# usamireko/WFL-ASR

Measured on AMD Instinct MI355X. Metric: audio_seconds_labeled_per_sec_per_node, higher is better.
Workload: dtype bf16; 1 GPU; BASELINE configs[1]: openai/whisper-base + 2 Conformer blocks, 16 x 30 s clips per GPU; clips_per_gpu=16, frames_per_clip=1500, tags=141, parallelism=clip-sharded dp1, launch=eager, batches_in_flight=2

## Files before the change

### include/wfl_asr.h

```cpp
#ifndef WFL_ASR_H
#define WFL_ASR_H

#include <stdint.h>

#ifdef __cplusplus
extern "C" {
#endif

typedef struct wfl_model wfl_model;

#define WFL_ENC_WHISPER 0
#define WFL_ENC_WAVLM 1
#define WFL_ENC_NONE 2

#define WFL_ABI_VERSION 2

typedef struct wfl_arch {
  int32_t abi_version;
  int32_t encoder_type;
  int32_t d_model;
  int32_t enc_layers;
  int32_t enc_heads;
  int32_t enc_ffn;
  int32_t n_mels;
// ... 63 lines not shown
int32_t wfl_head(wfl_model* m, const float* hidden, int32_t B, int32_t T, const int32_t* lang_id, int32_t lang_mode,
                 float threshold, void* workspace, int64_t workspace_bytes, int32_t* ids, int32_t* argmax, float* maxprob,
                 float* offsets, float* logits, int32_t* status, void* stream);

int32_t wfl_check(wfl_model* m, void* workspace, int64_t workspace_bytes, int32_t B, int32_t L, void* stream);


int32_t wfl_logmel(wfl_model* m, const float* wav, int64_t ldw, const int32_t* lens, int32_t B, int32_t L,
                   float* out, void* workspace, int64_t workspace_bytes, void* stream);

int32_t wfl_op_gemm(const void* A, int64_t lda, int32_t cin, int64_t tap_stride, const void* W, int32_t M, int32_t N,
                    int32_t K, int32_t n_valid, int32_t P, int32_t T, void* C, int64_t ldc, int64_t c_lead,
                    int32_t c_pitch, const float* bias, const void* res, int64_t ldres, float alpha, int32_t act,
                    int32_t glu, int32_t out_f32, void* stream);

int32_t wfl_op_gemm_split(const void* A_hi, const void* A_lo, int64_t lda, int32_t cin, int64_t tap_stride, const void* W3, int32_t M,
                          int32_t N, int32_t K, int32_t n_valid, int32_t P, int32_t T, void* C, void* C_lo, int64_t ldc,
                          int64_t c_lead, int32_t c_pitch, const float* bias, const void* res, const void* res_lo, int64_t ldres,
                          float alpha, int32_t act, int32_t glu, void* stream);

int32_t wfl_op_gemm_ln(const void* A, int64_t lda, const void* W, int32_t M, int32_t N, int32_t K, int32_t n_valid, int32_t P,
                       int32_t T, void* C, int64_t ldc, int64_t c_lead, int32_t c_pitch, const float* bias, const float* ln_s,
                       float ln_eps, int32_t act, void* stream);

int32_t wfl_op_attention(const void* QK, int64_t ldqk, int64_t lead, const void* V, int64_t ldv, void* O, int64_t ldo, int32_t B,
                         int32_t T, int32_t P, int32_t heads, int32_t d, void* stream);

int32_t wfl_op_attention_ex(const void* QK, const void* QK_lo, int64_t ldqk, int64_t lead, const void* V, const void* V_lo, int64_t ldv,
                            void* O, void* O_lo, int64_t ldo, int32_t B, int32_t T, int32_t P, int32_t heads, int32_t d, const float* bias,
                            const float* gate, const int32_t* clip_T, void* O8, void* O8_lo, int64_t ldo8, float o8_scale, int32_t* status,
// ... 218 lines not shown
```

### wfl-asr_amd/_lib.py

```python
from __future__ import annotations

import ctypes as C
import os

import numpy as np

PKG = os.path.dirname(os.path.abspath(__file__))
LIB_PATH = os.environ.get("WFL_LIB_PATH") or os.path.join(PKG, "libwfl_asr_hip.so")
ABI_VERSION = 2


class WflArch(C.Structure):
    _fields_ = [
        ("abi_version", C.c_int32), ("encoder_type", C.c_int32), ("d_model", C.c_int32), ("enc_layers", C.c_int32),
        ("enc_heads", C.c_int32), ("enc_ffn", C.c_int32), ("n_mels", C.c_int32), ("max_positions", C.c_int32),
        ("num_classes", C.c_int32), ("o_id", C.c_int32), ("num_languages", C.c_int32), ("lang_emb_dim", C.c_int32),
        ("enable_bilstm", C.c_int32), ("bilstm_layers", C.c_int32), ("n_conformer", C.c_int32),
        ("conformer_heads", C.c_int32), ("conformer_ff_expansion", C.c_int32), ("conformer_kernel", C.c_int32),
        ("enable_dilated", C.c_int32), ("dilated_depth", C.c_int32), ("dilated_kernel", C.c_int32),
        ("wavlm_n_conv", C.c_int32), ("wavlm_conv_dim", C.c_int32 * 8), ("wavlm_conv_kernel", C.c_int32 * 8),
        ("wavlm_conv_stride", C.c_int32 * 8), ("wavlm_group_norm", C.c_int32), ("wavlm_conv_bias", C.c_int32),
        ("wavlm_stable_layer_norm", C.c_int32), ("wavlm_pos_conv_kernel", C.c_int32),
        ("wavlm_pos_conv_groups", C.c_int32), ("wavlm_num_buckets", C.c_int32), ("wavlm_max_distance", C.c_int32),
        ("wavlm_do_normalize", C.c_int32), ("fp8_weights", C.c_int32), ("mel_hop", C.c_int32), ("precision", C.c_int32), ("fp8_activations", C.c_int32),
# ... 12 lines not shown
    "wfl_create": (_I, [C.POINTER(WflArch), C.POINTER(_P)]),
    "wfl_destroy": (None, [_P]),
    "wfl_load_tensor": (_I, [_P, C.c_char_p, _P, C.POINTER(_L), _I]),
    "wfl_finalize": (_I, [_P]),
    "wfl_num_frames": (_I, [_P, _I]),
    "wfl_workspace_bytes": (_L, [_P, _I, _I]),
    "wfl_device": (_I, [_P]),
    "wfl_set_average_languages": (_I, [_P, _P, _I]),
    "wfl_forward": (_I, [_P, _P, _L, _P, _I, _I, _P, _I, _F, _P, _L, _P, _P, _P, _P, _P, _P, _P, _P]),
    "wfl_encode": (_I, [_P, _P, _L, _P, _I, _I, _P, _L, _P, _P]),
    "wfl_head_workspace_bytes": (_L, [_P, _I, _I]),
    "wfl_head": (_I, [_P, _P, _I, _I, _P, _I, _F, _P, _L, _P, _P, _P, _P, _P, _P, _P]),
    "wfl_check": (_I, [_P, _P, _L, _I, _I, _P]),
    "wfl_logmel": (_I, [_P, _P, _L, _P, _I, _I, _P, _P, _L, _P]),
    "wfl_op_gemm": (_I, [_P, _L, _I, _L, _P, _I, _I, _I, _I, _I, _I, _P, _L, _L, _I, _P, _P, _L, _F, _I, _I, _I, _P]),
    "wfl_op_gemm_split": (_I, [_P, _P, _L, _I, _L, _P, _I, _I, _I, _I, _I, _I, _P, _P, _L, _L, _I, _P, _P, _P, _L, _F, _I, _I, _P]),
    "wfl_op_gemm_ln": (_I, [_P, _L, _P, _I, _I, _I, _I, _I, _I, _P, _L, _L, _I, _P, _P, _F, _I, _P]),
    "wfl_op_gemm_mx": (_I, [_P, _P, _L, _P, _P, _P, _F, _I, _I, _I, _I, _I, _P, _L, _L, _I, _P, _P, _P, _P, _F, _I, _P, _P, _L, _F, _P, _P]),
    "wfl_op_rows_fp8": (_I, [_P, _L, _P, _P, _P, _F, _L, _I, _I, _I, _I, _P, _P, _L, _P, _P]),
    "wfl_op_attention": (_I, [_P, _L, _L, _P, _L, _P, _L, _I, _I, _I, _I, _I, _P]),
    "wfl_op_attention_ex": (_I, [_P, _P, _L, _L, _P, _P, _L, _P, _P, _L, _I, _I, _I, _I, _I, _P, _P, _P, _P, _P, _L, _F, _P, _P]),
    "wfl_op_relpos_table": (_I, [_P, _P, _I, _I, _I, _P, _P]),
    "wfl_op_relpos_gate": (_I, [_P, _P, _L, _L, _I, _I, _I, _I, _I, _P, _P, _P, _P, _P]),
    "wfl_op_regroup": (_I, [_P, _I, _I, _I, _L, _L, _I, _I, _I, _P, _P, _P]),
    "wfl_op_wav_stats": (_I, [_P, _L, _P, _I, _I, _P, _P]),
    "wfl_op_clip_frames": (_I, [_P, _I, _I, _I, _P, _P, _I, _P, _P]),
    "wfl_op_conv0_scratch_bytes": (_L, [_I, _I, _I]),
    "wfl_op_conv0": (_I, [_P, _L, _P, _I, _I, _P, _P, _P, _P, _P, _I, _I, _P, _P, _L, _I, _I, _P, _L, _P]),
    "wfl_op_posconv": (_I, [_P, _L, _L, _I, _I, _I, _I, _I, _I, _P, _L, _P, _P, _P, _P, _P, _L, _P, _P]),
    "wfl_op_layernorm_act": (_I, [_P, _P, _L, _P, _P, _L, _P, _P, _F, _L, _I, _I, _I, _I, _I, _I, _P, _P]),
# ... 105 lines not shown
```

### wfl-asr_amd/csrc/common.h

```cpp
#pragma once
#include <hip/hip_runtime.h>
#include <stdint.h>

typedef __bf16 bf16_t;
typedef __attribute__((ext_vector_type(8))) __bf16 bf16x8;
typedef __attribute__((ext_vector_type(4))) __bf16 bf16x4;
typedef __attribute__((ext_vector_type(4))) float f32x4;
typedef __attribute__((ext_vector_type(16))) float f32x16;

#define WFL_ACT_NONE 0
#define WFL_ACT_GELU 1
#define WFL_ACT_RELU 2
#define WFL_ACT_SIGMOID 3

struct GemmArgs {
  const bf16_t* A;
  long lda;
  int cin;
  long tap_stride;
  int tap_wrap;
  long seg_off;
  const bf16_t* W;
  int M, N, K;
  int n_valid;
// ... 216 lines not shown
  bool need() {
    int d = 0;
    (void)hipGetDevice(&d);
    if ((mask >> (d & 31)) & 1u) return false;
    mask |= 1u << (d & 31);
    return true;
  }
};

int wfl_fail(int code, const char* msg);
int wfl_launch_gemm(const GemmArgs& a, hipStream_t s);
extern int g_wfl_gemm_kernel_id;
bool wfl_gemm_mx_takes(const GemmArgs& a);
int wfl_launch_gemm_mx(const GemmArgs& a, hipStream_t s);
bool wfl_gemm256_tri_takes(const GemmArgs& a);
bool wfl_gemm_stream_takes(const GemmArgs& a);
int wfl_launch_attention(const AttnArgs& a, hipStream_t s);
int wfl_launch_layernorm(const bf16_t* x, long ldx, bf16_t* y, long ldy, const float* g, const float* b, float eps,
                         long lead, int B, int P, int T, int C, hipStream_t s);
int wfl_launch_fill_i32(int* dst, long n, int value, hipStream_t s);
int wfl_launch_copy16(void* dst, const void* src, long bytes, hipStream_t s);
int wfl_launch_zero_halo(bf16_t* buf, long ld_bytes, long lead, int B, int P, int T, long tail_rows, hipStream_t s);
```

### wfl-asr_amd/csrc/gemm.hip

```cpp
#include "common.h"
#include <cstdlib>

#define BM 128
#define BN 128
#define BK 64
#define STAGE_BYTES (2 * BM * BK * 2)
#ifndef NSTAGE
#define NSTAGE 4
#endif
static_assert(NSTAGE >= 3 && NSTAGE <= 4, "the mid-iteration prefetch needs a ring of 3 or 4 K tiles");
#define EPI_BYTES (128 * 132 * 4)
#define LDS_BYTES (NSTAGE * STAGE_BYTES > EPI_BYTES ? NSTAGE * STAGE_BYTES : EPI_BYTES)

typedef __attribute__((address_space(1))) const void* gptr_t;
typedef __attribute__((address_space(3))) void* lptr_t;

#ifdef WFL_GEMM_STAMPS
#define STAMP(k) do { if (tid == 0 && p.stamps) p.stamps[(long)blockIdx.x * 8 + (k)] = __builtin_amdgcn_s_memrealtime(); } while (0)
#else
#define STAMP(k) do { } while (0)
#endif

static __device__ __forceinline__ void glds16(const bf16_t* g, char* l) {
  __builtin_amdgcn_global_load_lds((gptr_t)g, (lptr_t)l, 16, 0, 0);
// ... 290 lines not shown

int wfl_launch_gemm256(const GemmArgs& a, hipStream_t s);
int wfl_launch_gemm_stream(const GemmArgs& a, hipStream_t s);
bool wfl_gemm256_tri_takes(const GemmArgs& a);
bool wfl_gemm_stream_conv_takes(const GemmArgs& a);

static int tile_pref() {
  static int pref = -1;
  if (pref < 0) {
    const char* e = getenv("WFL_GEMM_TILE");
    pref = (e && atoi(e) == 128) ? 128 : 256;
  }
  return pref;
}

int wfl_launch_gemm(const GemmArgs& a, hipStream_t s) {
  if (a.M <= 0 || a.N <= 0 || a.N % BN || a.K <= 0 || a.K % BK || a.cin <= 0 || a.cin % BK || a.P <= 0 || a.P % 8 ||
      (!a.out_f32 && a.ldc % 8) || (a.res && a.ldres % 8) || (a.pos && a.ldpos % 8))
    return -1;
  if (a.a8 >= 2) {
    const int r = wfl_launch_gemm_mx(a, s);
    return r == 1 ? -1 : r;
  }
  if (tile_pref() == 256) {
    if (a.tap_wrap > 0 && wfl_gemm256_tri_takes(a) && !wfl_gemm_stream_conv_takes(a)) {
      static int tri_res = -1;
      if (tri_res < 0) { const char* e = getenv("WFL_TRI_RES"); tri_res = e ? atoi(e) : 1; }
      if (!a.res || tri_res) {
        const int r3 = wfl_launch_gemm256(a, s);
        if (r3 != 1) return r3;
      }
    }
    int r = wfl_launch_gemm_stream(a, s);
    if (r != 1) return r;
    if (a.ln_s || a.w8_scale) return -1;
    r = wfl_launch_gemm256(a, s);
    if (r != 1) return r;
  }
  if (a.ln_s || a.w8_scale) return -1;
  if (a.glu) {
    if (a.out_f32 || a.act != WFL_ACT_NONE) return -1;
    return launch_t<WFL_ACT_NONE, true, false>(a, s);
  }
  if (a.out_f32) {
    if (a.act == WFL_ACT_NONE) return launch_t<WFL_ACT_NONE, false, true>(a, s);
    if (a.act == WFL_ACT_SIGMOID) return launch_t<WFL_ACT_SIGMOID, false, true>(a, s);
// ... 11 lines not shown
```

### wfl-asr_amd/csrc/gemm_stream.hip

```cpp
#include "common.h"
#include <cstdlib>
#include <cstring>
#include <type_traits>

#define SBK 32
#ifndef SNST
#define SNST 4
#endif

#ifndef SNCU
#define SNCU 256
#endif

typedef __attribute__((address_space(1))) const void* sgptr_t;
typedef __attribute__((address_space(3))) void* slptr_t;
typedef __attribute__((ext_vector_type(2))) __bf16 bf16x2;

static __device__ __forceinline__ void sglds(const bf16_t* g, char* l) {
  __builtin_amdgcn_global_load_lds((sgptr_t)g, (slptr_t)l, 16, 0, 0);
}
static __device__ __forceinline__ int sswz(int row) { return (-(row >> 2)) & 3; }
static __device__ __forceinline__ int xswz(int row) { return ((row >> 2) & 1) << 1; }
#define XROT_ROWS 223
template <int N>
static __device__ __forceinline__ void wait_vm() { asm volatile("s_waitcnt vmcnt(%0)" ::"n"(N) : "memory"); }

#ifdef WFL_GEMM_STAMPS
#define SSTAMP(k) do { if (tid == 0 && p.stamps) { p.stamps[(long)blockIdx.x * 8 + (k)] = __builtin_amdgcn_s_memrealtime(); \
    if ((k) == 1) p.stamps[(long)blockIdx.x * 8 + 5] = __builtin_amdgcn_s_memtime(); \
    if ((k) == 2) p.stamps[(long)blockIdx.x * 8 + 6] = __builtin_amdgcn_s_memtime(); } } while (0)
#else
#define SSTAMP(k) do { } while (0)
#endif

template <int ACT, int MT, bool RES, int LNF, bool STATS, bool CONV, bool W8 = false, bool A8 = false, bool OUT8 = false, bool NOLO = false, bool ROT = false>
__global__ __launch_bounds__(512) void gemm_stream_kernel(GemmArgs p) {
  static_assert(!NOLO || CONV, "only the conv mode has an optional low half");
  static_assert(!ROT || CONV, "only the conv mode rotates frame fragments");
  static_assert(!CONV || (MT == 6 && !RES && LNF == 0 && !STATS), "conv mode: 192-row tiles, plain epilogue");
  static_assert(!W8 || (!CONV && MT == 6), "fp8 weights: plain 192-row mode");
  static_assert(!A8 || (!W8 && !CONV && MT == 6 && LNF == 0 && !STATS), "fp8 x fp8: the plain 192-row mode, no LayerNorm folding");
  static_assert(!OUT8 || (A8 && !RES), "fp8 output: the fp8 x fp8 kernel, no residual");
  constexpr int BMV = MT * 32;
#ifdef WFL_LAB_STB32
  constexpr int STB = 512 * SBK * 2;
  constexpr int WOFF = 256 * SBK * 2;
#else
  constexpr int STB = CONV ? 256 * SBK * 2 : BMV * SBK * 2 + 256 * SBK * (W8 ? 1 : 2);
  constexpr int WOFF = CONV ? 0 : BMV * SBK * 2;
#endif
  constexpr int AEXT = 224 * SBK * 2;
  constexpr int AOFF = SNST * STB;
  constexpr bool LOUT = RES || (CONV && !NOLO);
  constexpr int NSTORE = (LOUT ? 4 : 2) * MT + (STATS ? MT : 0);
  constexpr int SROW = 4;
  extern __shared__ __attribute__((aligned(16))) char smem[];
  float* stat_lds = (float*)(smem + SNST * STB + (CONV ? 2 * AEXT : 0));
  const int tid = threadIdx.x;
  const int lane = tid & 63;
  const int wid = __builtin_amdgcn_readfirstlane(tid >> 6);
  const int grp = wid >> 2, wq = wid & 3;
  const int g = lane >> 4, c = lane & 15;
  const int G = gridDim.x;

  SSTAMP(0);
  const int tiles_n = p.N / 256;
  const int tiles_m = (p.M + BMV - 1) / BMV;
  const int ntiles = tiles_m * tiles_n;
  const int nk = p.K / SBK;
// ... 132 lines not shown
      else if (SNST >= 5 && younger >= 3) { if (with_stores) wait_vm<3 * (L) + NSTORE>(); else wait_vm<3 * (L)>(); }  \
      else if (younger >= 2) { if (with_stores) wait_vm<2 * (L) + NSTORE>(); else wait_vm<2 * (L)>(); }              \
      else if (younger == 1) { if (with_stores) wait_vm<(L) + NSTORE>(); else wait_vm<(L)>(); }                      \
      else { if (with_stores) wait_vm<NSTORE>(); else wait_vm<0>(); }                                                \
    } while (0)
    if (CONV || two_x) WFL_WAITY(L2X); else WFL_WAITY(L1X);
#undef WFL_WAITY
  };

  int w_off[4];
#pragma unroll
  for (int v = 0; v < 4; ++v) {
#ifdef WFL_LAB_NOPERM
    const int r = wn + 16 * v + c;
#else
    const int r = wn + 32 * (v >> 1) + 8 * (c >> 2) + 4 * (v & 1) + (c & 3);
#endif
    w_off[v] = W8 ? WOFF + (r >> 3) * 256 + ((((r & 7) * 4 + g) ^ (((r >> 3) & 1) << 1) ^ (((r >> 4) & 1) << 4)) << 3)
                  : WOFF + r * 64 + ((g ^ sswz(r)) << 4);
  }
  const int x_off = wm * 64 + c * 64 + ((g ^ sswz(c)) << 4);

  f32x4 acc[MT][4];
#pragma unroll
  for (int u = 0; u < MT; ++u)
#pragma unroll
    for (int v = 0; v < 4; ++v) acc[u][v] = (f32x4){0.f, 0.f, 0.f, 0.f};
  float sa1 = 0.f, sa2 = 0.f, sb1 = 0.f, sb2 = 0.f;

  auto epilogue = [&](int m0, int n0) __attribute__((always_inline)) {
    const int nb = n0 + wn + 8 * g;
    constexpr int FCOL = ROT ? MT : 1, FROW = ROT ? 1 : 16;
    int mrow0 = m0 + wm + FCOL * c;
    int sidx_w = (((grp * 4 + wq) * (MT * 16)) + c) * 2, sidx_g = ((grp * 4 * (MT * 16)) + c) * 2, sidx_l = (grp * (MT * 16) + c) * 2;
    asm volatile("" : "+v"(mrow0), "+v"(sidx_w), "+v"(sidx_g), "+v"(sidx_l));
    f32x4 bj[4], sj[4], cj[(W8 || A8) ? 4 : 1];
#pragma unroll
    for (int h = 0; h < 2; ++h)
#pragma unroll
      for (int q = 0; q < 2; ++q) {
#ifdef WFL_ABL_EPI_NOLOAD
        bj[2 * h + q] = (f32x4){0.f, 0.f, 0.f, 0.f};
        if (LNF) sj[2 * h + q] = (f32x4){1.f, 1.f, 1.f, 1.f};
        if (W8 || A8) cj[2 * h + q] = (f32x4){1.f, 1.f, 1.f, 1.f};
#else
        bj[2 * h + q] = p.bias ? *(const f32x4*)(p.bias + nb + 32 * h + 4 * q) : (f32x4){0.f, 0.f, 0.f, 0.f};
        if (LNF) sj[2 * h + q] = *(const f32x4*)(p.ln_s + nb + 32 * h + 4 * q);
        if (W8 || A8) cj[2 * h + q] = *(const f32x4*)(p.w8_scale + nb + 32 * h + 4 * q);
#endif
      }
    float sa[A8 ? MT : 1];
    if (A8) {
#pragma unroll
      for (int u = 0; u < MT; ++u) {
        int m = mrow0 + FROW * u;
        m = m < p.M ? m : p.M - 1;
        sa[u] = p.a8_scale ? p.a8_scale[p.a8_lead + m] : p.a8_static;
      }
    }
    int P_ = p.P, cpitch = p.c_pitch;
    asm volatile("" : "+s"(P_), "+s"(cpitch));
    const float invP = __builtin_amdgcn_rcpf((float)P_);
    int orow[MT];
#pragma unroll
    for (int u = 0; u < MT; ++u) {
      const int m = mrow0 + FROW * u;
      int b = (int)((float)m * invP);
      int t = m - b * P_;
      if (t < 0) { t += P_; --b; }
      if (t >= P_) { t -= P_; ++b; }
      orow[u] = (m < p.M && t < p.T) ? (int)p.c_lead + b * cpitch + t : -1;
    }
    if (p.clip_T) {
#pragma unroll
      for (int u = 0; u < MT; ++u)
        if (orow[u] >= 0) {
          const int m = mrow0 + FROW * u;
          int b = (int)((float)m * invP);
          int t = m - b * P_;
          if (t < 0) { t += P_; --b; }
          if (t >= P_) { t -= P_; ++b; }
          if (t >= p.clip_T[b]) orow[u] = -1;
        }
    }
    constexpr int RING = 3;
    bf16x8 rr[RES ? RING : 1][2], rl[RES ? RING : 1][2];
    const bf16_t* res_lo = p.res_lo ? p.res_lo : p.res;
    const float lo_scale = p.res_lo ? 1.f : 0.f;
    auto load_res = [&](int u, int slot) __attribute__((always_inline)) {
      const long r = orow[u] >= 0 ? orow[u] : p.c_lead;
#pragma unroll
      for (int h = 0; h < 2; ++h) {
#ifdef WFL_ABL_EPI_NOLOAD
        rr[slot][h] = (bf16x8){0, 0, 0, 0, 0, 0, 0, 0}; rl[slot][h] = rr[slot][h]; (void)r;
#else
        rr[slot][h] = *(const bf16x8*)(p.res + r * p.ldres + nb + 32 * h);
        rl[slot][h] = *(const bf16x8*)(res_lo + r * p.ldres + nb + 32 * h);
#endif
      }
    };
    if (RES) {
#pragma unroll
      for (int u = 0; u < RING && u < MT; ++u) load_res(u, u);
    }
    float mu[LNF ? MT : 1], rs[LNF ? MT : 1];
    if (LNF == 1) {
#pragma unroll
      for (int u = 0; u < MT; ++u) {
        const float2 s = *(const float2*)(stat_lds + sidx_l + u * 32);
        mu[u] = s.x;
        rs[u] = s.y;
      }
    }
    if (LNF == 2) {
      f32x4 sp[MT][2];
#pragma unroll
      for (int u = 0; u < MT; ++u) {
        int m = mrow0 + FROW * u;
// ... 14 lines not shown
        mu[u] = mean;
        rs[u] = rsqrtf(fmaxf(__builtin_fmaf(-mean, mean, ex2), 0.f) + p.ln_eps);
      }
    }
    char* trash = (char*)p.trash + lane * 16;
#ifdef WFL_ABL_EPI_NOSTORE
#define WFL_KEEP(k) false
#else
#define WFL_KEEP(k) (k)
#endif
    float t1 = 0.f, t2 = 0.f;
    float amax8 = 0.f;
#pragma unroll
    for (int u = 0; u < MT; ++u) {
      __builtin_amdgcn_sched_barrier(0);
#pragma unroll
      for (int h = 0; h < 2; ++h) {
        float x[8];
#pragma unroll
        for (int q = 0; q < 2; ++q)
#pragma unroll
          for (int e = 0; e < 4; ++e) {
            float v = acc[u][2 * h + q][e];
            if (W8 || A8) v *= cj[2 * h + q][e];
            if (A8) v *= sa[u];
            if (LNF) v = (v - mu[u] * sj[2 * h + q][e]) * rs[u];
            if (ACT == WFL_ACT_GELU) {
              x[4 * q + e] = v + bj[2 * h + q][e];
              if (e & 1) {
                const f32x2 y = gelu_erf2((f32x2){x[4 * q + e - 1], x[4 * q + e]});
                x[4 * q + e - 1] = y[0]; x[4 * q + e] = y[1];
              }
              continue;
            }
            v = apply_act<ACT>(v + bj[2 * h + q][e]);
            if (RES) v = (bf2f(rr[u % RING][h][4 * q + e]) + lo_scale * bf2f(rl[u % RING][h][4 * q + e])) + p.alpha * v;
            x[4 * q + e] = v;
          }
        bf16x8 o;
#pragma unroll
        for (int e = 0; e < 8; ++e) o[e] = f2bf(x[e]);
        const bool keep = orow[u] >= 0 && nb + 32 * h < p.n_valid;
        if (OUT8) {
          int w0 = 0, w1 = 0;
          const float keepf = keep ? 1.f : 0.f;
#pragma unroll
          for (int e = 0; e < 8; ++e) {
            const float y = x[e] * p.c8_inv_scale;
            amax8 = fmaxf(amax8, fabsf(y) * keepf);
            x[e] = fminf(fmaxf(y, -448.f), 448.f);
          }
          w0 = __builtin_amdgcn_cvt_pk_fp8_f32(x[0], x[1], w0, false); w0 = __builtin_amdgcn_cvt_pk_fp8_f32(x[2], x[3], w0, true);
          w1 = __builtin_amdgcn_cvt_pk_fp8_f32(x[4], x[5], w1, false); w1 = __builtin_amdgcn_cvt_pk_fp8_f32(x[6], x[7], w1, true);
// ... 15 lines not shown
        }
        if (STATS) {
#pragma unroll
          for (int e = 0; e < 8; ++e) { const float r = bf2f(o[e]); t1 += r; t2 = fmaf(r, r, t2); }
        }
      }
      if (STATS) {
        t1 += __shfl_xor(t1, 16); t2 += __shfl_xor(t2, 16);
        t1 += __shfl_xor(t1, 32); t2 += __shfl_xor(t2, 32);
        if (g == 0) *(float2*)(stat_lds + sidx_w + u * 32) = float2{t1, t2};
        t1 = t2 = 0.f;
      }
#pragma unroll
      for (int v = 0; v < 4; ++v) acc[u][v] = (f32x4){0.f, 0.f, 0.f, 0.f};
      if (RES && u + RING < MT) load_res(u + RING, u % RING);
    }
    if (OUT8 && p.err) {
      if (__builtin_amdgcn_ballot_w64(amax8 > 448.f) && lane == 0) atomicOr(p.err, 2u);
    }
    if (STATS) {
      unsigned* cnt = (unsigned*)(stat_lds + 8 * (MT * 16) * 2) + grp;
      __builtin_amdgcn_s_waitcnt(0xC07F);
      unsigned ticket = 0;
      if (lane == 0) ticket = atomicAdd(cnt, 1u);
      ticket = __builtin_amdgcn_readfirstlane(ticket);
      const bool last = ticket == 3;
      if (last && lane == 0) *cnt = 0;
#pragma unroll
      for (int u = 0; u < MT; ++u) {
        float a1 = 0.f, a2 = 0.f;
// ... 185 lines not shown
#pragma unroll
    for (int kt = 1; kt < SNST - 2; ++kt) step_general(kt, std::false_type{});
    if (grp) steps_steady(std::true_type{}); else steps_steady(std::false_type{});
    for (int kt = nk - SNST > SNST - 2 ? nk - SNST : SNST - 2; kt < nk; ++kt) step_general(kt, std::false_type{});
    pm0 = m0; pn0 = n0;
    have_prev = true;
  }
  SSTAMP(2);
  SSTAMP(3);
  if (have_prev) epilogue(pm0, pn0);
  if (LNF == 1 && !grp) __builtin_amdgcn_s_barrier();
  SSTAMP(4);
#undef SSB
}

template <int ACT, int MT, bool RES, int LNF, bool STATS, bool CONV = false, bool W8 = false, bool A8 = false, bool OUT8 = false, bool NOLO = false, bool ROT = false>
static int launch_stream(const GemmArgs& a, hipStream_t s) {
  constexpr int BMV = MT * 32;
#ifdef WFL_LAB_STB32
  constexpr int lds = SNST * 512 * SBK * 2 + 8 * (MT * 16) * 2 * 4 + 64;
#else
  constexpr int lds = (CONV ? SNST * 256 * SBK * 2 + 2 * 224 * SBK * 2 : SNST * (BMV * SBK * 2 + 256 * SBK * (W8 ? 1 : 2))) + 8 * (MT * 16) * 2 * 4 + 64;
#endif
  const int tiles = ((a.M + BMV - 1) / BMV) * (a.N / 256);
  auto k = gemm_stream_kernel<ACT, MT, RES, LNF, STATS, CONV, W8, A8, OUT8, NOLO, ROT>;
  static WflOncePerDevice attr_once;
  if (attr_once.need()) {
    if (hipFuncSetAttribute((const void*)k, hipFuncAttributeMaxDynamicSharedMemorySize, lds) != hipSuccess) return -2;
  }
  g_wfl_gemm_kernel_id = CONV ? 6 : ((W8 || A8) ? 7 : (MT == 6 ? 1 : 5));
  hipLaunchKernelGGL(k, dim3(tiles < SNCU ? tiles : SNCU), dim3(512), lds, s, a);
  return hipGetLastError() == hipSuccess ? 0 : -3;
}

template <int ACT, bool RES, int LNF, bool STATS = false>
static int launch_stream_mt(const GemmArgs& a, hipStream_t s) {
  static int forced = -1;
  if (forced < 0) { const char* e = getenv("WFL_GEMM_BM"); forced = e ? atoi(e) : 0; }
#ifdef WFL_STREAM_MT8
  if (forced == 256) return launch_stream<ACT, 8, RES, LNF, STATS>(a, s);
// ... 18 lines not shown
  if (!g.c_lo) {
    switch (g.act) {
      case WFL_ACT_NONE: return launch_stream<WFL_ACT_NONE, 6, false, 0, false, true, false, false, false, true, ROT>(g, s);
      case WFL_ACT_GELU: return launch_stream<WFL_ACT_GELU, 6, false, 0, false, true, false, false, false, true, ROT>(g, s);
      case WFL_ACT_RELU: return launch_stream<WFL_ACT_RELU, 6, false, 0, false, true, false, false, false, true, ROT>(g, s);
    }
    return 1;
  }
  switch (g.act) {
    case WFL_ACT_NONE: return launch_stream<WFL_ACT_NONE, 6, false, 0, false, true, false, false, false, false, ROT>(g, s);
    case WFL_ACT_GELU: return launch_stream<WFL_ACT_GELU, 6, false, 0, false, true, false, false, false, false, ROT>(g, s);
    case WFL_ACT_RELU: return launch_stream<WFL_ACT_RELU, 6, false, 0, false, true, false, false, false, false, ROT>(g, s);
  }
  return 1;
}
bool wfl_gemm_stream_takes(const GemmArgs& a) {
  static int off = -1;
  if (off < 0) { const char* e = getenv("WFL_GEMM_NO_STREAM"); off = e && atoi(e) ? 1 : 0; }
  if (off) return false;
#ifdef WFL_LAB_NOSTREAM
  return false;
#endif
  if (a.glu || a.out_f32 || a.pos || a.clip_bias) return false;
  if (a.a8 >= 2) return false;
  if (a.tap_wrap > 0 && (a.ln_s || a.w8_scale || a.a8)) return false;
  if (a.c_lo && !a.res && !wfl_gemm_stream_conv(a)) return false;
  if (a.w8_scale && (a.cin < a.K || a.K % 64)) return false;
  if (a.a8 && (!a.w8_scale || a.ln_s || a.stats_out || a.stats_in || a.K % 128 || a.lda % 16 || a.K / 64 < 8 || (a.c8 && (a.res || a.ldc8 % 8))))
    return false;
  if (a.c8 && !a.a8) return false;
  if (a.N % 256 || a.K % SBK || a.cin % SBK || a.K / SBK < 8 || a.n_valid % 8) return false;
  if (a.stats_out && (!a.res || a.N / 256 > 4)) return false;
  if (a.stats_in && (!a.ln_s || a.stats_nsl <= 0 || a.stats_nsl > 4)) return false;
  if (a.res && a.act != WFL_ACT_NONE) return false;
  if (a.ln_s && (a.res || a.cin < a.K || (a.act != WFL_ACT_NONE && a.act != WFL_ACT_GELU))) return false;
  if (a.act == WFL_ACT_SIGMOID) return false;
  return true;
}


bool wfl_gemm_stream_conv_takes(const GemmArgs& a) { return wfl_gemm_stream_takes(a) && wfl_gemm_stream_conv(a); }

int wfl_launch_gemm_stream(const GemmArgs& a, hipStream_t s) {
  if (!wfl_gemm_stream_takes(a)) return 1;
  static void* trash[32] = {nullptr};
  int dev = 0;
  (void)hipGetDevice(&dev);
  dev &= 31;
  if (!trash[dev]) {
    if (hipMalloc(&trash[dev], 4096) != hipSuccess) return -2;
  }
  GemmArgs g = a;
  g.trash = trash[dev];
  g.ln_k_pow2 = (g.K & (g.K - 1)) == 0;
  g.ln_inv_k = g.ln_k_pow2 ? 1.0f / (float)g.K : 0.f;
  if (g.a8) {
    g.K /= 2; g.cin = g.K; g.lda /= 2;
    if (g.c8) return g.act == WFL_ACT_GELU ? launch_stream<WFL_ACT_GELU, 6, false, 0, false, false, false, true, true>(g, s) : -1;
    if (g.res) return g.act == WFL_ACT_NONE ? launch_stream<WFL_ACT_NONE, 6, true, 0, false, false, false, true>(g, s) : -1;
    if (g.act == WFL_ACT_NONE) return launch_stream<WFL_ACT_NONE, 6, false, 0, false, false, false, true>(g, s);
    return -1;
  }
  if (g.w8_scale) {
    if (g.ln_s && g.stats_in) {
      if (g.act == WFL_ACT_NONE) return launch_stream<WFL_ACT_NONE, 6, false, 2, false, false, true>(g, s);
      if (g.act == WFL_ACT_GELU) return launch_stream<WFL_ACT_GELU, 6, false, 2, false, false, true>(g, s);
      return -1;
    }
    if (g.res && !g.ln_s && g.act == WFL_ACT_NONE)
      return g.stats_out ? launch_stream<WFL_ACT_NONE, 6, true, 0, true, false, true>(g, s)
// ... 35 lines not shown
```

### wfl-asr_amd/csrc/model.hip

```cpp
#include "common.h"
#include "../../include/wfl_asr.h"

#include <cmath>
#include <cstdint>
#include <cstdio>
#include <cstring>
#include <map>
#include <set>
#include <string>
#include <vector>

int wfl_launch_logmel(const LogmelArgs& a, bf16_t* out, long ldo, long lead, int P, float* ref_out, hipStream_t s, bf16_t* out_lo = nullptr);
int wfl_launch_precise_finish(const PreciseFinishArgs& a, hipStream_t s);
int wfl_launch_melpower(const LogmelArgs& a, int hop, bf16_t* out, long ldo, long lead, int P, int split, int shift, hipStream_t s);

int wfl_launch_tag_decide(const TagArgs& a, hipStream_t s);
int wfl_launch_f32_to_rows(const float* in, bf16_t* x, long ldx, long lead, int B, int P, int T, int C, hipStream_t s, int split,
                           int shift, bf16_t* x_lo = nullptr);

int wfl_launch_lstm(LstmArgs a, void* exchange, hipStream_t s);

int wfl_launch_wav_stats(const float* wav, long ldw, int B, int L, double* stats, hipStream_t s, const int* lens = nullptr);
int wfl_launch_conv0(const Conv0Args& a, int group_norm, hipStream_t s);
int wfl_launch_clip_frames(const int* lens, int B, int L, int n, const int* kernel, const int* stride, int min_len, int* out, hipStream_t s);
// ... 1265 lines not shown
    void* const C = c.C;
    if (C == stats_for) stats_for = nullptr;
    const int B = r.M / r.P;
    const bf16_t* A_lo = lo_in(A);
    static int fused_on = -1;
    if (fused_on < 0) { const char* e = getenv("WFL_PRECISE_FUSED"); fused_on = e ? atoi(e) : 1; }
    static int pos_fused = -1;
    if (pos_fused < 0) { const char* e = getenv("WFL_PRECISE_POS_FUSED"); pos_fused = e ? atoi(e) : 1; }
    if (fused_on && W.W3 && A_lo && lo_of(C)) {
      GemmArgs g = gemm_args(A, lda, W, r, c, o);
      g.tap_wrap = W.K / g.cin; g.seg_off = (long)(A_lo - A);
      g.W = W.W3; g.K = 3 * W.K;
      g.res_lo = o.res ? lo_in(o.res) : nullptr;
      g.c_lo = lo_of(C);
      if (o.pos) g.pos_lo = (o.pos == m->pos) ? m->pos_lo : nullptr;
      if (!o.pos || (pos_fused && g.pos_lo && !o.glu && wfl_gemm256_tri_takes(g) && !wfl_gemm_stream_takes(g))) {
        mark_lo(C, true);
        launch_timed(g, 3.0 * 2.0 * (double)B * r.T * (double)W.n_valid * (double)W.K, "precision high, one-launch form: ");
        return;
      }
    }
    if ((long)r.M * W.N > p.hp32_floats) { rc = fail(-1, "precision high: the fp32 accumulator is too small for this launch"); return; }
    float* acc = (float*)(ws + p.hp32);
    for (int pass = 0; pass < 3; ++pass) {
      if (pass == 2 && !A_lo) break;
      GemmArgs g = gemm_args(pass == 2 ? A_lo : A, lda, W, r, {acc, W.N, 0, r.P}, partial_product(o));
      g.W = pass == 1 ? W.W_lo : W.W; g.n_valid = W.N; g.bias = nullptr; g.acc_f32 = pass > 0 ? 1 : 0;
      if (!launch_timed(g, 2.0 * (double)B * r.T * (double)W.n_valid * (double)W.K, "precision high, pass " + std::to_string(pass) + ": "))
        return;
    }
    PreciseFinishArgs f{};
// ... 677 lines not shown
}

int32_t wfl_op_gemm(const void* A, int64_t lda, int32_t cin, int64_t tap_stride, const void* W, int32_t M, int32_t N,
                    int32_t K, int32_t n_valid, int32_t P, int32_t T, void* C, int64_t ldc, int64_t c_lead, int32_t c_pitch,
                    const float* bias, const void* res, int64_t ldres, float alpha, int32_t act, int32_t glu,
                    int32_t out_f32, void* stream) {
  GemmArgs g{};
  g.A = (const bf16_t*)A; g.lda = lda; g.cin = cin > 0 ? cin : K; g.tap_stride = tap_stride;
  g.W = (const bf16_t*)W; g.M = M; g.N = N; g.K = K; g.n_valid = n_valid; g.P = P; g.T = T;
  g.C = C; g.ldc = ldc; g.c_lead = c_lead; g.c_pitch = c_pitch; g.bias = bias;
  g.res = (const bf16_t*)res; g.ldres = ldres; g.alpha = alpha; g.act = act; g.glu = glu; g.out_f32 = out_f32;
  const int r = wfl_launch_gemm(g, (hipStream_t)stream);
  return r ? fail(r, "wfl_op_gemm: invalid arguments or launch failure (" + std::to_string(r) + ")") : 0;
}

int32_t wfl_op_gemm_ln(const void* A, int64_t lda, const void* W, int32_t M, int32_t N, int32_t K, int32_t n_valid, int32_t P,
                       int32_t T, void* C, int64_t ldc, int64_t c_lead, int32_t c_pitch, const float* bias, const float* ln_s,
                       float ln_eps, int32_t act, void* stream) {
  if (!ln_s) return fail(-1, "wfl_op_gemm_ln: ln_s is required");
  GemmArgs g{};
  g.A = (const bf16_t*)A; g.lda = lda; g.cin = K; g.tap_stride = 0;
  g.W = (const bf16_t*)W; g.M = M; g.N = N; g.K = K; g.n_valid = n_valid; g.P = P; g.T = T;
  g.C = C; g.ldc = ldc; g.c_lead = c_lead; g.c_pitch = c_pitch; g.bias = bias; g.alpha = 1.f; g.act = act;
  g.ln_s = ln_s; g.ln_eps = ln_eps;
  const int r = wfl_launch_gemm(g, (hipStream_t)stream);
  return r ? fail(r, "wfl_op_gemm_ln: shape not supported by the LayerNorm-folding kernel or launch failure (" + std::to_string(r) + ")") : 0;
}

int32_t wfl_op_gemm_split(const void* A_hi, const void* A_lo, int64_t lda, int32_t cin, int64_t tap_stride, const void* W3, int32_t M,
                          int32_t N, int32_t K, int32_t n_valid, int32_t P, int32_t T, void* C, void* C_lo, int64_t ldc, int64_t c_lead,
// ... 194 lines not shown
```

Measured before the change: 135,400 audio-s/s.

## Route GLU, fp32-out, positional-add and per-clip-bias GEMMs to the streaming kernel

Adds four epilogue variants to the streaming 192-row GEMM kernel: GLU gating with an interleaved weight-row permutation, fp32 output, GELU plus positional-embedding add, and per-clip bias gathered by index. GEMMs carrying these options used to be refused by the streaming path and fell back to the older tiled kernels; they can now use the pipelined stream kernel. It also factors tri-kernel routing into a shared predicate and adds a wfl_op_gemm_ex entry point for testing. The cost is more template instances and register pressure in the epilogue, plus the risk that the GLU row permutation or bias indexing is wrong.

```diff
diff --git a/include/wfl_asr.h b/include/wfl_asr.h
--- a/include/wfl_asr.h
+++ b/include/wfl_asr.h
@@ -101,6 +101,12 @@
                     int32_t c_pitch, const float* bias, const void* res, int64_t ldres, float alpha, int32_t act,
                     int32_t glu, int32_t out_f32, void* stream);
 
+int32_t wfl_op_gemm_ex(const void* A, int64_t lda, int32_t cin, int64_t tap_stride, const void* W, int32_t M, int32_t N, int32_t K,
+                       int32_t n_valid, int32_t P, int32_t T, void* C, void* C_lo, int64_t ldc, int64_t c_lead, int32_t c_pitch,
+                       const float* bias, const void* res, int64_t ldres, float alpha, int32_t act, int32_t glu, int32_t out_f32,
+                       const void* pos, const void* pos_lo, int64_t ldpos, const float* clip_bias, const int32_t* clip_idx, int32_t clip_ld,
+                       int32_t tap_wrap, int64_t seg_off, void* stream);
+
 int32_t wfl_op_gemm_split(const void* A_hi, const void* A_lo, int64_t lda, int32_t cin, int64_t tap_stride, const void* W3, int32_t M,
                           int32_t N, int32_t K, int32_t n_valid, int32_t P, int32_t T, void* C, void* C_lo, int64_t ldc,
                           int64_t c_lead, int32_t c_pitch, const float* bias, const void* res, const void* res_lo, int64_t ldres,
diff --git a/wfl-asr_amd/_lib.py b/wfl-asr_amd/_lib.py
--- a/wfl-asr_amd/_lib.py
+++ b/wfl-asr_amd/_lib.py
@@ -50,6 +50,8 @@
     "wfl_check": (_I, [_P, _P, _L, _I, _I, _P]),
     "wfl_logmel": (_I, [_P, _P, _L, _P, _I, _I, _P, _P, _L, _P]),
     "wfl_op_gemm": (_I, [_P, _L, _I, _L, _P, _I, _I, _I, _I, _I, _I, _P, _L, _L, _I, _P, _P, _L, _F, _I, _I, _I, _P]),
+    "wfl_op_gemm_ex": (_I, [_P, _L, _I, _L, _P, _I, _I, _I, _I, _I, _I, _P, _P, _L, _L, _I, _P, _P, _L, _F, _I, _I, _I, _P, _P, _L, _P, _P, _I,
+                            _I, _L, _P]),
     "wfl_op_gemm_split": (_I, [_P, _P, _L, _I, _L, _P, _I, _I, _I, _I, _I, _I, _P, _P, _L, _L, _I, _P, _P, _P, _L, _F, _I, _I, _P]),
     "wfl_op_gemm_ln": (_I, [_P, _L, _P, _I, _I, _I, _I, _I, _I, _P, _L, _L, _I, _P, _P, _F, _I, _P]),
     "wfl_op_gemm_mx": (_I, [_P, _P, _L, _P, _P, _P, _F, _I, _I, _I, _I, _I, _P, _L, _L, _I, _P, _P, _P, _P, _F, _I, _P, _P, _L, _F, _P, _P]),
diff --git a/wfl-asr_amd/csrc/common.h b/wfl-asr_amd/csrc/common.h
--- a/wfl-asr_amd/csrc/common.h
+++ b/wfl-asr_amd/csrc/common.h
@@ -254,6 +254,7 @@
 bool wfl_gemm_mx_takes(const GemmArgs& a);
 int wfl_launch_gemm_mx(const GemmArgs& a, hipStream_t s);
 bool wfl_gemm256_tri_takes(const GemmArgs& a);
+bool wfl_gemm_routes_to_tri(const GemmArgs& a);
 bool wfl_gemm_stream_takes(const GemmArgs& a);
 int wfl_launch_attention(const AttnArgs& a, hipStream_t s);
 int wfl_launch_layernorm(const bf16_t* x, long ldx, bf16_t* y, long ldy, const float* g, const float* b, float eps,
diff --git a/wfl-asr_amd/csrc/gemm.hip b/wfl-asr_amd/csrc/gemm.hip
--- a/wfl-asr_amd/csrc/gemm.hip
+++ b/wfl-asr_amd/csrc/gemm.hip
@@ -328,22 +328,31 @@
   return pref;
 }
 
+static bool args_ok(const GemmArgs& a) {
+  return !(a.M <= 0 || a.N <= 0 || a.N % BN || a.K <= 0 || a.K % BK || a.cin <= 0 || a.cin % BK || a.P <= 0 || a.P % 8 ||
+           (!a.out_f32 && a.ldc % 8) || (a.res && a.ldres % 8) || (a.pos && a.ldpos % 8));
+}
+
+bool wfl_gemm_routes_to_tri(const GemmArgs& a) {
+  if (!args_ok(a) || a.a8 >= 2 || tile_pref() != 256) return false;
+  if (a.tap_wrap <= 0 || !wfl_gemm256_tri_takes(a) || wfl_gemm_stream_conv_takes(a)) return false;
+  static int tri_res = -1;
+  if (tri_res < 0) { const char* e = getenv("WFL_TRI_RES"); tri_res = e ? atoi(e) : 1; }
+  return !a.res || tri_res;
+}
+
 int wfl_launch_gemm(const GemmArgs& a, hipStream_t s) {
-  if (a.M <= 0 || a.N <= 0 || a.N % BN || a.K <= 0 || a.K % BK || a.cin <= 0 || a.cin % BK || a.P <= 0 || a.P % 8 ||
-      (!a.out_f32 && a.ldc % 8) || (a.res && a.ldres % 8) || (a.pos && a.ldpos % 8))
-    return -1;
+  if (!args_ok(a)) return -1;
+  if (a.pos_lo && !wfl_gemm_routes_to_tri(a)) return -1;
   if (a.a8 >= 2) {
     const int r = wfl_launch_gemm_mx(a, s);
     return r == 1 ? -1 : r;
   }
   if (tile_pref() == 256) {
-    if (a.tap_wrap > 0 && wfl_gemm256_tri_takes(a) && !wfl_gemm_stream_conv_takes(a)) {
-      static int tri_res = -1;
-      if (tri_res < 0) { const char* e = getenv("WFL_TRI_RES"); tri_res = e ? atoi(e) : 1; }
-      if (!a.res || tri_res) {
-        const int r3 = wfl_launch_gemm256(a, s);
-        if (r3 != 1) return r3;
-      }
+    if (wfl_gemm_routes_to_tri(a)) {
+      const int r3 = wfl_launch_gemm256(a, s);
+      if (r3 != 1) return r3;
+      if (a.pos_lo) return -1;
     }
     int r = wfl_launch_gemm_stream(a, s);
     if (r != 1) return r;
diff --git a/wfl-asr_amd/csrc/gemm_stream.hip b/wfl-asr_amd/csrc/gemm_stream.hip
--- a/wfl-asr_amd/csrc/gemm_stream.hip
+++ b/wfl-asr_amd/csrc/gemm_stream.hip
@@ -33,8 +33,16 @@
 #define SSTAMP(k) do { } while (0)
 #endif
 
-template <int ACT, int MT, bool RES, int LNF, bool STATS, bool CONV, bool W8 = false, bool A8 = false, bool OUT8 = false, bool NOLO = false, bool ROT = false>
+#define EPI_NONE 0
+#define EPI_CLIP 1
+#define EPI_POS 2
+#define EPI_GLU 3
+#define EPI_F32 4
+template <int ACT, int MT, bool RES, int LNF, bool STATS, bool CONV, bool W8 = false, bool A8 = false, bool OUT8 = false, bool NOLO = false, bool ROT = false, int EPI = EPI_NONE>
 __global__ __launch_bounds__(512) void gemm_stream_kernel(GemmArgs p) {
+  static_assert(EPI == EPI_NONE || (MT == 6 && !RES && LNF == 0 && !STATS && !CONV && !W8 && !A8), "epilogue forms: the plain 192-row bf16 mode");
+  static_assert(EPI != EPI_GLU || ACT == WFL_ACT_NONE, "GLU has no activation of its own");
+  constexpr bool CLIP = EPI == EPI_CLIP, POS = EPI == EPI_POS, GLU = EPI == EPI_GLU, F32 = EPI == EPI_F32;
   static_assert(!NOLO || CONV, "only the conv mode has an optional low half");
   static_assert(!ROT || CONV, "only the conv mode rotates frame fragments");
   static_assert(!CONV || (MT == 6 && !RES && LNF == 0 && !STATS), "conv mode: 192-row tiles, plain epilogue");
@@ -51,8 +59,8 @@
 #endif
   constexpr int AEXT = 224 * SBK * 2;
   constexpr int AOFF = SNST * STB;
-  constexpr bool LOUT = RES || (CONV && !NOLO);
-  constexpr int NSTORE = (LOUT ? 4 : 2) * MT + (STATS ? MT : 0);
+  constexpr bool LOUT = RES || (CONV && !NOLO) || CLIP || POS;
+  constexpr int NSTORE = GLU ? MT : F32 ? 4 * MT : (LOUT ? 4 : 2) * MT + (STATS ? MT : 0);
   constexpr int SROW = 4;
   extern __shared__ __attribute__((aligned(16))) char smem[];
   float* stat_lds = (float*)(smem + SNST * STB + (CONV ? 2 * AEXT : 0));
@@ -215,7 +223,8 @@
 #ifdef WFL_LAB_NOPERM
     const int r = wn + 16 * v + c;
 #else
-    const int r = wn + 32 * (v >> 1) + 8 * (c >> 2) + 4 * (v & 1) + (c & 3);
+    const int r = GLU ? wn + 32 * (c >> 3) + 16 * (v & 1) + 8 * ((c >> 2) & 1) + 4 * (v >> 1) + (c & 3)
+                      : wn + 32 * (v >> 1) + 8 * (c >> 2) + 4 * (v & 1) + (c & 3);
 #endif
     w_off[v] = W8 ? WOFF + (r >> 3) * 256 + ((((r & 7) * 4 + g) ^ (((r >> 3) & 1) << 1) ^ (((r >> 4) & 1) << 4)) << 3)
                   : WOFF + r * 64 + ((g ^ sswz(r)) << 4);
@@ -230,7 +239,8 @@
   float sa1 = 0.f, sa2 = 0.f, sb1 = 0.f, sb2 = 0.f;
 
   auto epilogue = [&](int m0, int n0) __attribute__((always_inline)) {
-    const int nb = n0 + wn + 8 * g;
+    const int nb = GLU ? (n0 >> 1) + (wn >> 1) + 8 * g : n0 + wn + 8 * g;
+    const int nbw = n0 + wn + 32 * (g >> 1) + 8 * (g & 1);
     constexpr int FCOL = ROT ? MT : 1, FROW = ROT ? 1 : 16;
     int mrow0 = m0 + wm + FCOL * c;
     int sidx_w = (((grp * 4 + wq) * (MT * 16)) + c) * 2, sidx_g = ((grp * 4 * (MT * 16)) + c) * 2, sidx_l = (grp * (MT * 16) + c) * 2;
@@ -245,7 +255,8 @@
         if (LNF) sj[2 * h + q] = (f32x4){1.f, 1.f, 1.f, 1.f};
         if (W8 || A8) cj[2 * h + q] = (f32x4){1.f, 1.f, 1.f, 1.f};
 #else
-        bj[2 * h + q] = p.bias ? *(const f32x4*)(p.bias + nb + 32 * h + 4 * q) : (f32x4){0.f, 0.f, 0.f, 0.f};
+        if (GLU) bj[2 * h + q] = p.bias ? *(const f32x4*)(p.bias + nbw + 4 * h + 16 * q) : (f32x4){0.f, 0.f, 0.f, 0.f};
+        else bj[2 * h + q] = p.bias ? *(const f32x4*)(p.bias + nb + 32 * h + 4 * q) : (f32x4){0.f, 0.f, 0.f, 0.f};
         if (LNF) sj[2 * h + q] = *(const f32x4*)(p.ln_s + nb + 32 * h + 4 * q);
         if (W8 || A8) cj[2 * h + q] = *(const f32x4*)(p.w8_scale + nb + 32 * h + 4 * q);
 #endif
@@ -263,6 +274,7 @@
     asm volatile("" : "+s"(P_), "+s"(cpitch));
     const float invP = __builtin_amdgcn_rcpf((float)P_);
     int orow[MT];
+    int tix[(CLIP || POS) ? MT : 1];
 #pragma unroll
     for (int u = 0; u < MT; ++u) {
       const int m = mrow0 + FROW * u;
@@ -271,6 +283,12 @@
       if (t < 0) { t += P_; --b; }
       if (t >= P_) { t -= P_; ++b; }
       orow[u] = (m < p.M && t < p.T) ? (int)p.c_lead + b * cpitch + t : -1;
+      if (POS) tix[u] = orow[u] >= 0 ? t : 0;
+      if (CLIP) tix[u] = m < p.M ? b : 0;
+    }
+    if (CLIP) {
+#pragma unroll
+      for (int u = 0; u < MT; ++u) tix[u] = p.clip_idx[tix[u]];
     }
     if (p.clip_T) {
 #pragma unroll
@@ -284,8 +302,20 @@
           if (t >= p.clip_T[b]) orow[u] = -1;
         }
     }
-    constexpr int RING = 3;
-    bf16x8 rr[RES ? RING : 1][2], rl[RES ? RING : 1][2];
+    constexpr int RING = POS ? MT : 3;
+    bf16x8 rr[(RES || POS) ? RING : 1][2], rl[RES ? RING : 1][2];
+    f32x4 cbr[CLIP ? RING : 1][4];
+    auto load_epi = [&](int u, int slot) __attribute__((always_inline)) {
+#pragma unroll
+      for (int h = 0; h < 2; ++h) {
+        const int n1 = nb + 32 * h < p.n_valid ? nb + 32 * h : 0;
+        if (POS) rr[slot][h] = *(const bf16x8*)(p.pos + (long)tix[u] * p.ldpos + n1);
+        if (CLIP) {
+#pragma unroll
+          for (int q = 0; q < 2; ++q) cbr[slot][2 * h + q] = *(const f32x4*)(p.clip_bias + (long)tix[u] * p.clip_ld + n1 + 4 * q);
+        }
+      }
+    };
     const bf16_t* res_lo = p.res_lo ? p.res_lo : p.res;
     const float lo_scale = p.res_lo ? 1.f : 0.f;
     auto load_res = [&](int u, int slot) __attribute__((always_inline)) {
@@ -303,6 +333,10 @@
     if (RES) {
 #pragma unroll
       for (int u = 0; u < RING && u < MT; ++u) load_res(u, u);
+    }
+    if (CLIP || POS) {
+#pragma unroll
+      for (int u = 0; u < RING && u < MT; ++u) load_epi(u, u);
     }
     float mu[LNF ? MT : 1], rs[LNF ? MT : 1];
     if (LNF == 1) {
@@ -347,6 +381,21 @@
 #pragma unroll
     for (int u = 0; u < MT; ++u) {
       __builtin_amdgcn_sched_barrier(0);
+      if (GLU) {
+        bf16x8 o;
+#pragma unroll
+        for (int jp = 0; jp < 2; ++jp)
+#pragma unroll
+          for (int e = 0; e < 4; ++e)
+            o[4 * jp + e] = f2bf((acc[u][2 * jp][e] + bj[2 * jp][e]) * sigmoidf_(acc[u][2 * jp + 1][e] + bj[2 * jp + 1][e]));
+        const bool keep = orow[u] >= 0 && nb < (p.n_valid >> 1);
+        char* dst = (char*)((bf16_t*)p.C + (long)orow[u] * p.ldc + nb);
+        dst = WFL_KEEP(keep) ? dst : trash;
+        *(bf16x8*)dst = o;
+#pragma unroll
+        for (int v = 0; v < 4; ++v) acc[u][v] = (f32x4){0.f, 0.f, 0.f, 0.f};
+        continue;
+      }
 #pragma unroll
       for (int h = 0; h < 2; ++h) {
         float x[8];
@@ -360,16 +409,37 @@
             if (LNF) v = (v - mu[u] * sj[2 * h + q][e]) * rs[u];
             if (ACT == WFL_ACT_GELU) {
               x[4 * q + e] = v + bj[2 * h + q][e];
+              if (CLIP) x[4 * q + e] += cbr[u % RING][2 * h + q][e];
               if (e & 1) {
                 const f32x2 y = gelu_erf2((f32x2){x[4 * q + e - 1], x[4 * q + e]});
                 x[4 * q + e - 1] = y[0]; x[4 * q + e] = y[1];
               }
               continue;
             }
-            v = apply_act<ACT>(v + bj[2 * h + q][e]);
+            v = v + bj[2 * h + q][e];
+            if (CLIP) v += cbr[u % RING][2 * h + q][e];
+            v = apply_act<ACT>(v);
             if (RES) v = (bf2f(rr[u % RING][h][4 * q + e]) + lo_scale * bf2f(rl[u % RING][h][4 * q + e])) + p.alpha * v;
             x[4 * q + e] = v;
           }
+        if (POS) {
+#pragma unroll
+          for (int e = 0; e < 8; ++e) x[e] += bf2f(rr[u % RING][h][e]);
+        }
+        if (F32) {
+          const int n1 = nb + 32 * h;
+          const bool full = n1 + 8 <= p.n_valid && (p.ldc & 3) == 0;
+          float* o32 = (float*)p.C + (long)orow[u] * p.ldc + n1;
+          char* d32 = WFL_KEEP(orow[u] >= 0 && full) ? (char*)o32 : trash;
+          *(f32x4*)d32 = (f32x4){x[0], x[1], x[2], x[3]};
+          *(f32x4*)(WFL_KEEP(orow[u] >= 0 && full) ? d32 + 16 : d32) = (f32x4){x[4], x[5], x[6], x[7]};
+          if (WFL_KEEP(orow[u] >= 0 && !full && n1 < p.n_valid)) {
+#pragma unroll
+            for (int e = 0; e < 8; ++e)
+              if (n1 + e < p.n_valid) o32[e] = x[e];
+          }
+          continue;
+        }
         bf16x8 o;
 #pragma unroll
         for (int e = 0; e < 8; ++e) o[e] = f2bf(x[e]);
@@ -415,6 +485,7 @@
 #pragma unroll
       for (int v = 0; v < 4; ++v) acc[u][v] = (f32x4){0.f, 0.f, 0.f, 0.f};
       if (RES && u + RING < MT) load_res(u + RING, u % RING);
+      if ((CLIP || POS) && u + RING < MT) load_epi(u + RING, u % RING);
     }
     if (OUT8 && p.err) {
       if (__builtin_amdgcn_ballot_w64(amax8 > 448.f) && lane == 0) atomicOr(p.err, 2u);
@@ -630,7 +701,8 @@
 #undef SSB
 }
 
-template <int ACT, int MT, bool RES, int LNF, bool STATS, bool CONV = false, bool W8 = false, bool A8 = false, bool OUT8 = false, bool NOLO = false, bool ROT = false>
+template <int ACT, int MT, bool RES, int LNF, bool STATS, bool CONV = false, bool W8 = false, bool A8 = false, bool OUT8 = false, bool NOLO = false, bool ROT = false,
+          int EPI = EPI_NONE>
 static int launch_stream(const GemmArgs& a, hipStream_t s) {
   constexpr int BMV = MT * 32;
 #ifdef WFL_LAB_STB32
@@ -639,7 +711,7 @@
   constexpr int lds = (CONV ? SNST * 256 * SBK * 2 + 2 * 224 * SBK * 2 : SNST * (BMV * SBK * 2 + 256 * SBK * (W8 ? 1 : 2))) + 8 * (MT * 16) * 2 * 4 + 64;
 #endif
   const int tiles = ((a.M + BMV - 1) / BMV) * (a.N / 256);
-  auto k = gemm_stream_kernel<ACT, MT, RES, LNF, STATS, CONV, W8, A8, OUT8, NOLO, ROT>;
+  auto k = gemm_stream_kernel<ACT, MT, RES, LNF, STATS, CONV, W8, A8, OUT8, NOLO, ROT, EPI>;
   static WflOncePerDevice attr_once;
   if (attr_once.need()) {
     if (hipFuncSetAttribute((const void*)k, hipFuncAttributeMaxDynamicSharedMemorySize, lds) != hipSuccess) return -2;
@@ -688,6 +760,24 @@
   }
   return 1;
 }
+static int stream_epi_form(const GemmArgs& a) {
+  const int n = (a.glu ? 1 : 0) + (a.out_f32 ? 1 : 0) + (a.pos ? 1 : 0) + (a.clip_bias ? 1 : 0);
+  if (n == 0) return EPI_NONE;
+  const char* e = getenv("WFL_STREAM_EPI");
+  if (e && e[0] == '0' && !e[1]) return -1;
+  if (n != 1 || a.res || a.ln_s || a.w8_scale || a.a8 || a.c8 || a.stats_out || a.stats_in || a.acc_f32 || a.pos_lo) return -1;
+  if (a.n_valid <= 0 || a.n_valid > a.N) return -1;
+  if (a.out_f32) {
+    if (a.act != WFL_ACT_NONE || a.c_lo) return -1;
+    if (a.tap_wrap > 0 && a.K != 3 * a.tap_wrap * a.cin) return -1;
+    return wfl_gemm_stream_conv(a) ? -1 : EPI_F32;
+  }
+  if (a.tap_wrap > 0 || wfl_gemm_stream_conv(a)) return -1;
+  if (a.glu) return (a.act == WFL_ACT_NONE && !a.c_lo && a.n_valid % 16 == 0) ? EPI_GLU : -1;
+  if (a.pos) return (a.act == WFL_ACT_GELU && a.ldpos % 8 == 0) ? EPI_POS : -1;
+  return (a.act == WFL_ACT_NONE && a.clip_idx && a.clip_ld % 4 == 0) ? EPI_CLIP : -1;
+}
+
 bool wfl_gemm_stream_takes(const GemmArgs& a) {
   static int off = -1;
   if (off < 0) { const char* e = getenv("WFL_GEMM_NO_STREAM"); off = e && atoi(e) ? 1 : 0; }
@@ -695,15 +785,16 @@
 #ifdef WFL_LAB_NOSTREAM
   return false;
 #endif
-  if (a.glu || a.out_f32 || a.pos || a.clip_bias) return false;
+  const int epi = stream_epi_form(a);
+  if (epi < 0) return false;
   if (a.a8 >= 2) return false;
   if (a.tap_wrap > 0 && (a.ln_s || a.w8_scale || a.a8)) return false;
-  if (a.c_lo && !a.res && !wfl_gemm_stream_conv(a)) return false;
+  if (a.c_lo && !a.res && !wfl_gemm_stream_conv(a) && epi != EPI_CLIP && epi != EPI_POS) return false;
   if (a.w8_scale && (a.cin < a.K || a.K % 64)) return false;
   if (a.a8 && (!a.w8_scale || a.ln_s || a.stats_out || a.stats_in || a.K % 128 || a.lda % 16 || a.K / 64 < 8 || (a.c8 && (a.res || a.ldc8 % 8))))
     return false;
   if (a.c8 && !a.a8) return false;
-  if (a.N % 256 || a.K % SBK || a.cin % SBK || a.K / SBK < 8 || a.n_valid % 8) return false;
+  if (a.N % 256 || a.K % SBK || a.cin % SBK || a.K / SBK < 8 || (a.n_valid % 8 && epi != EPI_F32)) return false;
   if (a.stats_out && (!a.res || a.N / 256 > 4)) return false;
   if (a.stats_in && (!a.ln_s || a.stats_nsl <= 0 || a.stats_nsl > 4)) return false;
   if (a.res && a.act != WFL_ACT_NONE) return false;
@@ -728,6 +819,12 @@
   g.trash = trash[dev];
   g.ln_k_pow2 = (g.K & (g.K - 1)) == 0;
   g.ln_inv_k = g.ln_k_pow2 ? 1.0f / (float)g.K : 0.f;
+  switch (stream_epi_form(g)) {
+    case EPI_CLIP: return launch_stream<WFL_ACT_NONE, 6, false, 0, false, false, false, false, false, false, false, EPI_CLIP>(g, s);
+    case EPI_POS: return launch_stream<WFL_ACT_GELU, 6, false, 0, false, false, false, false, false, false, false, EPI_POS>(g, s);
+    case EPI_GLU: return launch_stream<WFL_ACT_NONE, 6, false, 0, false, false, false, false, false, false, false, EPI_GLU>(g, s);
+    case EPI_F32: return launch_stream<WFL_ACT_NONE, 6, false, 0, false, false, false, false, false, false, false, EPI_F32>(g, s);
+  }
   if (g.a8) {
     g.K /= 2; g.cin = g.K; g.lda /= 2;
     if (g.c8) return g.act == WFL_ACT_GELU ? launch_stream<WFL_ACT_GELU, 6, false, 0, false, false, false, true, true>(g, s) : -1;
diff --git a/wfl-asr_amd/csrc/model.hip b/wfl-asr_amd/csrc/model.hip
--- a/wfl-asr_amd/csrc/model.hip
+++ b/wfl-asr_amd/csrc/model.hip
@@ -1303,7 +1303,7 @@
       g.res_lo = o.res ? lo_in(o.res) : nullptr;
       g.c_lo = lo_of(C);
       if (o.pos) g.pos_lo = (o.pos == m->pos) ? m->pos_lo : nullptr;
-      if (!o.pos || (pos_fused && g.pos_lo && !o.glu && wfl_gemm256_tri_takes(g) && !wfl_gemm_stream_takes(g))) {
+      if (!o.pos || (pos_fused && g.pos_lo && !o.glu && wfl_gemm_routes_to_tri(g))) {
         mark_lo(C, true);
         launch_timed(g, 3.0 * 2.0 * (double)B * r.T * (double)W.n_valid * (double)W.K, "precision high, one-launch form: ");
         return;
@@ -2011,6 +2011,34 @@
   return r ? fail(r, "wfl_op_gemm: invalid arguments or launch failure (" + std::to_string(r) + ")") : 0;
 }
 
+int32_t wfl_op_gemm_ex(const void* A, int64_t lda, int32_t cin, int64_t tap_stride, const void* W, int32_t M, int32_t N, int32_t K,
+                       int32_t n_valid, int32_t P, int32_t T, void* C, void* C_lo, int64_t ldc, int64_t c_lead, int32_t c_pitch,
+                       const float* bias, const void* res, int64_t ldres, float alpha, int32_t act, int32_t glu, int32_t out_f32,
+                       const void* pos, const void* pos_lo, int64_t ldpos, const float* clip_bias, const int32_t* clip_idx, int32_t clip_ld,
+                       int32_t tap_wrap, int64_t seg_off, void* stream) {
+  if (!A || !W || !C) return fail(-1, "wfl_op_gemm_ex: null argument");
+  if (M <= 0 || N <= 0 || K <= 0 || P <= 0 || T < 0 || n_valid <= 0 || n_valid > N) return fail(-1, "wfl_op_gemm_ex: bad shape");
+  if (cin > 0 && K % cin) return fail(-1, "wfl_op_gemm_ex: K must be a whole number of taps");
+  if (C_lo && (out_f32 || glu)) return fail(-1, "wfl_op_gemm_ex: a low half goes with a plain bf16 output only");
+  if (pos && (ldpos < n_valid || ldpos % 8)) return fail(-1, "wfl_op_gemm_ex: ldpos must be a multiple of 8, at least n_valid");
+  if (pos_lo && !pos) return fail(-1, "wfl_op_gemm_ex: pos_lo without pos");
+  if (!clip_bias != !clip_idx) return fail(-1, "wfl_op_gemm_ex: clip_bias and clip_idx go together");
+  if (clip_bias && (clip_ld < n_valid || clip_ld % 4)) return fail(-1, "wfl_op_gemm_ex: clip_ld must be a multiple of 4, at least n_valid");
+  if (tap_wrap < 0 || (tap_wrap > 0 && (cin <= 0 || (int64_t)3 * tap_wrap * cin != K)))
+    return fail(-1, "wfl_op_gemm_ex: tap_wrap needs K = 3 segments of tap_wrap taps of cin channels");
+  GemmArgs g{};
+  g.A = (const bf16_t*)A; g.lda = lda; g.cin = cin > 0 ? cin : K; g.tap_stride = tap_stride;
+  g.W = (const bf16_t*)W; g.M = M; g.N = N; g.K = K; g.n_valid = n_valid; g.P = P; g.T = T;
+  g.C = C; g.c_lo = (bf16_t*)C_lo; g.ldc = ldc; g.c_lead = c_lead; g.c_pitch = c_pitch; g.bias = bias;
+  g.res = (const bf16_t*)res; g.ldres = ldres; g.alpha = alpha; g.act = act; g.glu = glu; g.out_f32 = out_f32;
+  g.pos = (const bf16_t*)pos; g.pos_lo = (const bf16_t*)pos_lo; g.ldpos = ldpos;
+  g.clip_bias = clip_bias; g.clip_idx = clip_idx; g.clip_ld = clip_ld;
+  g.tap_wrap = tap_wrap; g.seg_off = seg_off;
+  g.ln_eps = 1e-5f;
+  const int r = wfl_launch_gemm(g, (hipStream_t)stream);
+  return r ? fail(r, "wfl_op_gemm_ex: invalid arguments or launch failure (" + std::to_string(r) + ")") : 0;
+}
+
 int32_t wfl_op_gemm_ln(const void* A, int64_t lda, const void* W, int32_t M, int32_t N, int32_t K, int32_t n_valid, int32_t P,
                        int32_t T, void* C, int64_t ldc, int64_t c_lead, int32_t c_pitch, const float* bias, const float* ln_s,
                        float ln_eps, int32_t act, void* stream) {
```

Measured after the change: 136,400 audio-s/s (median of 6 runs). About the same (+0.7%).
